# deepsphere/deepsphere-cosmo-tf2

Measured on AMD Instinct MI355X. Metric: Mpix*channels/s Chebyshev-conv fwd, nside=1024 K=5 F=64; HBM roofline %, higher is better.
Workload: dtype f32 (recurrence f32; contraction 3-pass split-bf16 MFMA with f32 accumulate; precision 'bf16x3' = the layer default for 64 input channels)

## Files before the change

deepsphere-cosmo-tf2_amd/csrc/cheb_fused.hip:

```cpp
#include <stdio.h>
#include <stdlib.h>
#include <string.h>

#include <algorithm>

#include "cheb_istrip_kernel.h"
#include "cheb_tiles.h"

namespace dsph {

void fused_images_begin(const dsph_plan* plan, const void* ws, uint64_t key, bool keep) {
  FusedPlan* fp = plan->fused;
  if (!fp || !ws) return;
  std::lock_guard<std::mutex> lock(fp->img_mu);
  if (fp->images.size() > 16384 && fp->images.find(ws) == fp->images.end()) fp->images.clear();
  FusedPlan::Images& im = fp->images[ws];
  if (!keep || im.key != key) { im.key = key; im.mask = 0; }
}
bool fused_images_claim(const dsph_plan* plan, const void* ws, uint32_t bit) {
  FusedPlan* fp = plan->fused;
  if (!fp || !ws) return true;
  std::lock_guard<std::mutex> lock(fp->img_mu);
  auto it = fp->images.find(ws);
  if (it == fp->images.end()) return true;
// ... 388 lines not shown

static int launch_strips(const FusedRequest& rq, const Route& rt, const WeightImages& img, const LaunchBase& base) {
  const dsph_plan* plan = rq.plan;
  const FusedTiles& ft = rt.ft;
  if (rt.strips == Strips::quad) {
    QStripLaunch qs;
    static_cast<LaunchBase&>(qs) = base;
    qs.wimg = rq.ws + img.qstrip;
    qs.strips = ft.q5.d_strips;
    qs.tab = ft.q5.d_tab;
    qs.prefix = ft.q5.d_prefix;
    qs.tape_rows = ft.q5.tape_rows;
    qs.nstrips = ft.q5.n; qs.Fin = rq.Fin; qs.Fout = rq.Fout;
    qs.f16 = rq.precision == DSPH_PREC_F16X3;
    qs.f16_xexp = plan->opt.f16_xexp;
    qs.prep_weights = fused_images_claim(plan, rq.ws, IMG_QSTRIP);
    return launch_cheb_qstrip(qs, rq.stream);
  }
  if (rt.strips == Strips::pairs) {
    StripLaunch st;
    static_cast<LaunchBase&>(st) = base;
    st.wimg = rq.ws + img.strip;
    st.pairs = ft.d_pairs;
    st.npairs = ft.n_pairs; st.Fin = rq.Fin; st.Fout = rq.Fout; st.K = rq.K; st.precision = struct_arithmetic(rq.precision);
    st.prep_weights = fused_images_claim(plan, rq.ws, IMG_STRIP);
    return launch_cheb_strip(st, rq.stream);
  }
  IStripLaunch is;
  static_cast<LaunchBase&>(is) = base;
  is.wimg = rq.ws + img.istrip;
// ... 389 lines not shown
```

deepsphere-cosmo-tf2_amd/csrc/cheb_qstrip.hip:

```cpp
#include <math.h>
#include <stdio.h>
#include <stdlib.h>

#include <algorithm>
#include <vector>

#include "cheb_qstrip_kernel.h"
#include "dsphere_wfrag.h"

namespace dsph {

__global__ __launch_bounds__(256) void qstrip_wprep_kernel(const float* __restrict__ w, unsigned char* __restrict__ out, int Fin,
                                                           int Fout, int cheb, int ld, int f16) {
  constexpr int K = 5;
  const int blk = blockIdx.x;
  const int kb = blk & 1, lev = (blk >> 1) % 3, oq = ((blk >> 1) / 3) & 3, role = (blk >> 1) / 12;
  const int j = role == 0 ? K - 1 - lev : 1 - lev;
  const bool have = role == 0 || lev < 2;
  float sc = qs_wsign(cheb != 0, j) * ((cheb != 0 && j == 0) ? 2.f : 1.f);
  if (f16) {
    const float pw = qt_wimg_pow2(w, Fin * K, Fout, ld);
    sc *= pw;
    if (blk == 0 && threadIdx.x == 0) *reinterpret_cast<float*>(out + (size_t)2 * 4 * 3 * 2 * 2 * QS_FRAG) = 1.f / pw;
  }
// ... 29 lines not shown
  return qtape_split(num_cu, tape_rows, N, mean_height, QS_RUNIN, grid, pieces, wg_per_piece);
}

size_t qstrip_wimg_bytes() { return (size_t)2 * 4 * 3 * 2 * 2 * QS_FRAG + 256; }

int launch_cheb_qstrip(const QStripLaunch& s, hipStream_t stream) {
  if (s.prep_weights) {
    hipLaunchKernelGGL(qstrip_wprep_kernel, dim3(2 * 4 * 3 * 2), dim3(256), 0, stream, s.w, s.wimg, (int)s.Fin, (int)s.Fout, s.cheb ? 1 : 0,
                       (int)s.ld, s.f16 ? 1 : 0);
    DSPH_HIP(hipGetLastError());
  }
  QStripArgs a;
  a.Fin = s.Fin;
  a.Fout = s.Fout;
  const int grid = qtape_forward_args(a, s, QS_RUNIN);
  void (*kern)(QStripArgs) = s.f16 ? (s.cheb ? cheb_qstrip5_kernel<true, true> : cheb_qstrip5_kernel<false, true>)
                                   : (s.cheb ? cheb_qstrip5_kernel<true, false> : cheb_qstrip5_kernel<false, false>);
#ifdef DSPH_QS_STAMPS
  static unsigned* d_stamps = nullptr;
  constexpr size_t NST = 8 * 4 * 10;
  if (!d_stamps) DSPH_HIP(hipMalloc(&d_stamps, NST * 4));
  DSPH_HIP(hipMemsetAsync(d_stamps, 0, NST * 4, stream));
  a.stamps = d_stamps;
#endif
  hipLaunchKernelGGL(kern, dim3(grid), dim3(QS_THREADS), 0, stream, a);
  DSPH_HIP(hipGetLastError());
#ifdef DSPH_QS_STAMPS
  if (getenv("DSPH_STAMPS_DUMP")) {
    std::vector<unsigned> h(NST);
    if (hipStreamSynchronize(stream) == hipSuccess && hipMemcpy(h.data(), d_stamps, NST * 4, hipMemcpyDeviceToHost) == hipSuccess)
      for (int w = 0; w < 8; ++w)
        for (int it = 0; it < 4; ++it) {
// ... 17 lines not shown
```

deepsphere-cosmo-tf2_amd/csrc/cheb_qstrip_kernel.h:

```cpp
#pragma once

#include <type_traits>

#include "cheb_qtape.h"

namespace dsph {

constexpr int QS_PX = 64;
constexpr int QS_D = 4;
constexpr int QS_USE = QS_PX - 2 * QS_D;
constexpr int QS_THREADS = 512;
constexpr int QS_RUNIN = 2 * QS_D + 1;

struct QStripArgs {
  const float* x;
  const float* bias;
  float* y;
  const unsigned char* wimg;
  const float* gvals8;
  const float* gdiag;
  const QStrip* strips;
  const int32_t* tab;
  const int32_t* prefix;
  int64_t x_rows, y_rows;
// ... 111 lines not shown
    qs_u12<INIT, NEG>(a0, a1, a2, a3, src.t[0][E], src.t[1][E], src.t[2][E], src.t[3][E], cw, cc, ce);                    \
    acc.t[0][E] = a0; acc.t[1][E] = a1; acc.t[2][E] = a2; acc.t[3][E] = a3;                                               \
  }
  if (e == 0) QS_UE(0)
  else if (e == 1) QS_UE(1)
  else if (e == 2) QS_UE(2)
  else QS_UE(3)
#undef QS_UE
}

#define QS_UPR 4
#define QS_UNIT qs_unit

__host__ __device__ constexpr float qs_wsign(bool cheb, int j) { return cheb && ((j & 3) >= 2) ? -1.f : 1.f; }

template <bool CHEB, bool F16>
__global__ __launch_bounds__(QS_THREADS, 2) void cheb_qstrip5_kernel(QStripArgs a) {
  constexpr int K = 5, D = QS_D, RING = K + 2;
#ifdef DSPH_QS_NOH1
  constexpr bool H1 = false;
#else
  constexpr bool H1 = CHEB;
#endif
  constexpr int ROWB = 2 * 2 * 4 * QS_FRAG;
  constexpr int RINGB = RING * ROWB;
  constexpr int HAND1 = 2 * 4 * QS_FRAG;
  constexpr int HANDB = 4 * HAND1;
  constexpr int CRING = K + 1;
  constexpr int CRINGB = CRING * QS_CROWB;
  constexpr int LDS_HAND = RINGB, LDS_C = RINGB + HANDB, LDS_FLAG = LDS_C + CRINGB;
  __shared__ __attribute__((aligned(16))) unsigned char smem[LDS_FLAG + 64];
// ... 30 lines not shown
  const unsigned x_goff = X_BY_H ? (unsigned)(2 * (lane >> 5) + (lane & 1)) * 16u
                                 : (unsigned)(lane >> 5) * 64u + (unsigned)(2 * ((lane >> 4) & 1) + (lane & 1)) * 16u;
  const unsigned x_loff = (unsigned)xt * QS_FRAG + (unsigned)(lane & 1) * 8u +
                          (X_BY_H ? (unsigned)(xpix + 16 * (lane >> 5)) * 16u : (unsigned)(xpix + 16 * (2 * (lane >> 5) + ((lane >> 4) & 1))) * 16u);
  auto tab_lane = [&](const QStrip& st, unsigned ci, int yrow) __attribute__((always_inline)) -> unsigned {
    return qt_tab_lane(a.tab, st, ci, min(max(yrow, st.ylo), st.yhi));
  };
  auto my_of = [&](int yrow) __attribute__((always_inline)) -> unsigned { return st_spread((unsigned)yrow & 15u) << 1; };
  auto my_next = [&](unsigned m) __attribute__((always_inline)) -> unsigned { return ((m | 0x55u) + 1u) & 0xaau; };
  auto xfetch = [&](const char* xmap, unsigned xrow, qs_f4 (&xv)[XN]) __attribute__((always_inline)) {
    if (QS_ABL & 8) {
#pragma unroll
      for (int i = 0; i < XN; ++i) xv[i] = qs_f4{0.f, 0.f, 0.f, 0.f};
      return;
    }
    const char* src = xmap + (size_t)(xrow * xrowb + x_goff);
#pragma unroll
    for (int i = 0; i < XN; ++i) xv[i] = *reinterpret_cast<const qs_f4*>(src + (X_BY_H ? 64 : 128) * i);
  };
  auto xw_wait = [&](qs_f4 (&xv)[XN]) __attribute__((always_inline)) {
    if (X_BY_H) asm volatile("" : "+v"(xv[0]), "+v"(xv[1]), "+v"(xv[XN - 2]), "+v"(xv[XN - 1]) : : "memory");
    else asm volatile("" : "+v"(xv[0]), "+v"(xv[1]) : : "memory");
  };
  auto xstore = [&](int slot, const qs_f4 (&xv)[XN]) __attribute__((always_inline)) {
    if (QS_ABL & 4096) {
#pragma unroll
      for (int i = 0; i < XN; ++i) asm volatile("" : : "v"(xv[i]));
      return;
    }
    unsigned char* q = smem + (unsigned)slot * ROWB + x_loff;
#pragma unroll
    for (int i = 0; i < XN; ++i) {
      const unsigned fo = X_BY_H ? (unsigned)(i >> 1) * (2 * 4 * QS_FRAG) + (unsigned)(i & 1) * (32u * 16u) : (unsigned)i * (2 * 4 * QS_FRAG);
      qs_u2 hi, lo;
#pragma unroll
      for (int j = 0; j < 2; ++j) {
        const float a0 = F16 ? xv[i][2 * j] * a.xsc : xv[i][2 * j], a1 = F16 ? xv[i][2 * j + 1] * a.xsc : xv[i][2 * j + 1];
        const qs_u2 hl = qt_split<F16>(a0, a1);
        hi[j] = hl[0];
        lo[j] = hl[1];
      }
      *reinterpret_cast<qs_u2*>(q + fo) = hi;
      *reinterpret_cast<qs_u2*>(q + fo + 4 * QS_FRAG) = lo;
    }
  };
  auto cfetch = [&](unsigned rid, qs_f4& cv, float& cd) __attribute__((always_inline)) { qt_cfetch(a.gvals8, a.gdiag, rid, q4, cv, cd); };
  auto cw_wait = [&](qs_f4& cv, float& cd) __attribute__((always_inline)) {
    asm volatile("" : "+v"(cv), "+v"(cd) : : "memory");
  };
  auto cstore = [&](int slot, qs_f4 cv, float cd) __attribute__((always_inline)) {
    if (CHEB) { cv = cv + cv; cd = cd + cd; }
    unsigned char* q = smem + LDS_C + (unsigned)slot * QS_CROWB + (unsigned)p * 16u + (unsigned)oq * 4u;
    if (q4 < 2) {
#pragma unroll
      for (int d = 0; d < 4; ++d) *reinterpret_cast<float*>(q + (unsigned)(1 + 4 * q4 + d) * 256u) = cv[d];
    }
    if (q4 == 2) *reinterpret_cast<float*>(q) = cd;
  };
  constexpr bool C_OFF = (QS_ABL & 1024) != 0;
  auto clo_read = [&](int slot) __attribute__((always_inline)) -> QCoefLo { return qt_clo_read<C_OFF>(smem + LDS_C, slot, p); };
  auto chi_read = [&](int slot) __attribute__((always_inline)) -> QCoefHi { return qt_chi_read<C_OFF>(smem + LDS_C, slot, p); };

#if QS_ABL & 512
#define QS_FRLOAD(P) (wr[0][0][0])
#else
#define QS_FRLOAD(P) (*reinterpret_cast<const qs_bf8*>(P))
#endif
#define QS_ORD_A(j) ((j) == 1 ? 1 : 0)
#define QS_ORD_B(j) ((j) == 0 ? 1 : 0)
#define QS_FR0(FADDR)                                                                                                     \
  _Pragma("unroll") for (int u = 0; u < 2; ++u) {                                                                         \
    fr[0][u][0] = QS_FRLOAD(smem + (FADDR) + (unsigned)u * QS_FRAG);                                                      \
    fr[0][u][1] = QS_FRLOAD(smem + (FADDR) + (unsigned)(4 + u) * QS_FRAG);                                                \
  }
#define QS_SETS(S0, S1, ROW, ZERO, WLEV, FADDR, NU, ...)                                                                  \
  _Pragma("unroll") for (int s = (S0); s < (S1); ++s) {                 \
    if (s + 1 < 4) {                                                                                                      \
      _Pragma("unroll") for (int u = 0; u < 2; ++u) {                                                                     \
        const unsigned fo = (unsigned)(((s + 1) >> 1) * 8 + ((s + 1) & 1) * 2 + u) * QS_FRAG;                             \
        fr[(s + 1) & 1][u][0] = QS_FRLOAD(smem + (FADDR) + fo);                                                           \
        fr[(s + 1) & 1][u][1] = QS_FRLOAD(smem + (FADDR) + fo + 4 * QS_FRAG);                                             \
      }                                                                                                                   \
    }                                                                                                                     \
    _Pragma("unroll") for (int j = 0; j < 3; ++j) {                                                                       \
      _Pragma("unroll") for (int u = 0; u < 2; ++u) {                                                                     \
        const int m = (s * 3 + j) * 2 + u;                                                                                \
        const int tt = (s & 1) * 2 + u;                                                                                   \
        const qs_bf8& wa_ = wr[WLEV][s >> 1][QS_ORD_A(j)];                                                                \
        const qs_bf8& bb_ = fr[s & 1][u][QS_ORD_B(j)];                                                                    \
        if ((ZERO) && s < 2 && j == 0) qs_m0<F16>((ROW).t[tt], wa_, bb_);                                                 \
        else qs_m<F16>((ROW).t[tt], wa_, bb_);                                                                            \
        _Pragma("unroll") for (int qq = (m * (NU)) / 18; qq < ((m + 1) * (NU)) / 18 && m < 18; ++qq) { __VA_ARGS__; }     \
      }                                                                                                                   \
    }                                                                                                                     \
  }
#define QS_CHAIN(ROW, ZERO, WLEV, FADDR, NU, TAIL, ...)                                                                   \
  {                                                                                                                       \
    QS_SETS(0, 3, ROW, ZERO, WLEV, FADDR, NU, __VA_ARGS__)                                                                \
// ... 10 lines not shown
#pragma unroll
      for (int kb = 0; kb < 2; ++kb)
#pragma unroll
        for (int h = 0; h < 2; ++h) wr[3][kb][h] = *reinterpret_cast<const qs_bf8*>(wp1 + (size_t)(kb * 2 + h) * QS_FRAG);
    }
    {
      const unsigned char* wp = a.wimg + ((size_t)(0 * 4 + oq) * 3) * (2 * 2 * QS_FRAG) + lane16;
#pragma unroll
      for (int l = 0; l < 3; ++l)
#pragma unroll
        for (int kb = 0; kb < 2; ++kb)
#pragma unroll
          for (int h = 0; h < 2; ++h) wr[l][kb][h] = *reinterpret_cast<const qs_bf8*>(wp + ((size_t)(l * 2 + kb) * 2 + h) * QS_FRAG);
    }
    int handed = 0;
    for (int64_t tr = tape.begin; tr < tape.end;) {
      QStrip st;
      tr += locate(tr, tape.end, st);
      for (int nq = wg.map0; nq < a.N; nq += a.wg_per_piece) {
      const int Xc = min(max(st.xs + 4 * p + oq, st.xlo), st.xhi);
      const int Xf = min(max(st.xs + 4 * xpix + xt, st.xlo), st.xhi);
      const int tc0 = max(st.xs, st.xlo) >> 4;
      const unsigned ciC = (unsigned)((Xc >> 4) - tc0), mXc = st_spread((unsigned)Xc & 15u);
      const unsigned ciF = (unsigned)((Xf >> 4) - tc0), mXf = st_spread((unsigned)Xf & 15u);
      const int T3 = ((st.y1 - st.y0) + 2 * D + 1 + 3) / 3;
      const char* __restrict__ xmap = reinterpret_cast<const char*>(a.x) + (size_t)nq * a.x_rows * xrowb;
      QRow R[2][3];
#pragma unroll
      for (int i = 0; i < 2; ++i)
#pragma unroll
        for (int s = 0; s < 3; ++s)
#pragma unroll
          for (int t = 0; t < 4; ++t) R[i][s].t[t] = qs_f4{0.f, 0.f, 0.f, 0.f};
      int ytop = st.y0 - D, slot_top = 0, cs_top = 0;
      qt_step_barrier();
      {
        qs_f4 cv, xv[XN];
        float cd;
        cfetch(qt_row_in(st, tab_lane(st, ciC, ytop - 1), mXc, ytop - 1), cv, cd);
        xfetch(xmap, qt_row_in(st, tab_lane(st, ciF, ytop), mXf, ytop), xv);
        cw_wait(cv, cd);
        cstore(CRING - 1, cv, cd);
        xw_wait(xv);
        xstore(0, xv);
      }
      unsigned bXf = tab_lane(st, ciF, ytop + 1), bXc = tab_lane(st, ciC, ytop);
      unsigned myX = my_of(ytop + 1), myC = my_of(ytop);
      qt_step_barrier();
      auto step = [&](auto ph_c) __attribute__((always_inline)) {
        constexpr int PH = decltype(ph_c)::value;
        constexpr int L0 = PH % 3, L1 = (PH + 1) % 3, L2 = (PH + 2) % 3;
        int snew = slot_top + 1;
        snew = snew == RING ? 0 : snew;
        auto slot_ix = [&](int back) __attribute__((always_inline)) -> int {
          int s = slot_top - back;
          s += s < 0 ? RING : 0;
          return s;
        };
        auto cslot_ix = [&](int back) __attribute__((always_inline)) -> int {
          int s = cs_top - back;
          s += s < 0 ? CRING : 0;
          return s;
        };
        QS_STAMP_DECL
        QS_STAMP(0);
        qs_f4 xv[XN];
        constexpr bool XLATE = H1;
        if (myX == 0) bXf = tab_lane(st, ciF, ytop + 1);
        if (myC == 0) bXc = tab_lane(st, ciC, ytop);
        if (!XLATE) xfetch(xmap, bXf + (mXf | myX), xv);
        const unsigned f0 = (unsigned)slot_top * ROWB + lane16, f1 = (unsigned)slot_ix(1) * ROWB + lane16, f2 = (unsigned)slot_ix(2) * ROWB + lane16;
        const unsigned f3 = (unsigned)slot_ix(3) * ROWB + lane16;
        constexpr bool N3 = CHEB;
        qs_bf8 fr[2][2][2];
        QCoefLo c3 = clo_read(cslot_ix(1));
        QS_FR0(f0)
        QCoefLo c2;
        QCoefHi c3h, c2h;
        qs_f4 cv;
        float cd;
        QS_CHAIN(R[0][L2], true, 0, f0, 2 * QS_UPR, { c2 = clo_read(cslot_ix(2)); QS_FR0(f1) },
                 { if (qq < QS_UPR) QS_UNIT<true, N3>(R[1][L2], R[0][L0], qq, QS_LO0(c3)); else QS_UNIT<false, N3>(R[1][L2], R[0][L1], qq - QS_UPR, QS_LO1(c3)); })
        qs_settle<9>(R[0][L2]);
        qs_settle<1>(R[1][L2]);
        QS_STAMP(1);
        QS_CHAIN(R[1][L2], false, 1, f1, 2 * QS_UPR, { c3h = chi_read(cslot_ix(1)); QS_FR0(f2) },
                 { if (qq < QS_UPR) QS_UNIT<!CHEB, false>(R[0][L0], R[1][L0], qq, QS_LO0(c2)); else QS_UNIT<false, false>(R[0][L0], R[1][L1], qq - QS_UPR, QS_LO1(c2)); })
        qs_settle<9>(R[1][L2]);
        qs_settle<1>(R[0][L0]);
        if (XLATE) xfetch(xmap, bXf + (mXf | myX), xv);
        QS_STAMP(2);
        QS_CHAIN(R[0][L0], false, 2, f2, QS_UPR, { c2h = chi_read(cslot_ix(2)); cfetch(bXc + (mXc | myC), cv, cd); if (H1) { QS_FR0(f3) } },
                 { QS_UNIT<false, N3>(R[1][L2], R[0][L2], qq, QS_HI(c3h)); })
        qs_settle<9>(R[0][L0]);
        qs_settle<1>(R[1][L2]);
        QS_STAMP(3);
        if (H1) {
          QS_CHAIN(R[1][L0], false, 3, f3, QS_UPR, {}, { QS_UNIT<false, false>(R[0][L0], R[1][L2], qq, QS_HI(c2h)); })
          qs_settle<9>(R[1][L0]);
        } else {
#pragma unroll
          for (int qq = 0; qq < QS_UPR; ++qq) QS_UNIT<false, false>(R[0][L0], R[1][L2], qq, QS_HI(c2h));
        }
        QS_STAMP(4);
        for (int spin = 0; flag_get() <= handed && spin < (1 << 22); ++spin) {}
        if (!(QS_ABL & 2048)) {
          unsigned char* hp = smem + hand;
#pragma unroll
          for (int t = 0; t < 4; ++t) {
            *reinterpret_cast<qs_f4*>(hp + t * QS_FRAG) = R[0][L0].t[t];
            if (CHEB) *reinterpret_cast<qs_f4*>(hp + (4 + t) * QS_FRAG) = R[1][L0].t[t];
          }
        }
        ++handed;
        QS_STAMP(5);
        xw_wait(xv);
        cw_wait(cv, cd);
        QS_STAMP(6);
        cstore(cs_top, cv, cd);
        xstore(snew, xv);
        QS_STAMP(7);
        slot_top = snew;
        cs_top = cs_top + 1 == CRING ? 0 : cs_top + 1;
        ++ytop;
        myX = my_next(myX);
        myC = my_next(myC);
        qt_step_barrier();
        QS_STAMP(8);
      };
      for (int t3 = 0; t3 < T3; ++t3) {
        step(std::integral_constant<int, 0>{});
        step(std::integral_constant<int, 1>{});
        step(std::integral_constant<int, 2>{});
      }
      }
    }
  } else {
    qs_bf8 wr[2][2][2];
    {
      const unsigned char* wp = a.wimg + ((size_t)(1 * 4 + oq) * 3) * (2 * 2 * QS_FRAG) + lane16;
#pragma unroll
// ... 23 lines not shown
      const int Xg = st.xs + 4 * p;
      const unsigned ciY = (unsigned)((min(max(Xg, st.xlo), st.xhi) >> 4) - tc0), mXg = st_spread((unsigned)Xg & 12u);
      const int cfirst = st.x0 - st.xs, clast = cfirst + st.w;
      const int T3 = ((st.y1 - st.y0) + 2 * D + 1 + 3) / 3;
      const char* __restrict__ xmap = reinterpret_cast<const char*>(a.x) + (size_t)nq * a.x_rows * xrowb;
      char* __restrict__ ymap = reinterpret_cast<char*>(a.y) + (size_t)nq * a.y_rows * yrowb;
      QRow R[2][3], Y;
#pragma unroll
      for (int i = 0; i < 2; ++i)
#pragma unroll
        for (int s = 0; s < 3; ++s)
#pragma unroll
          for (int t = 0; t < 4; ++t) R[i][s].t[t] = qs_f4{0.f, 0.f, 0.f, 0.f};
#pragma unroll
      for (int t = 0; t < 4; ++t) Y.t[t] = qs_f4{0.f, 0.f, 0.f, 0.f};
      int ytop = st.y0 - D, slot_top = 0, cs_top = 0;
      qt_step_barrier();
      if (!X_BY_H) {
        qs_f4 xv[XN];
        xfetch(xmap, qt_row_in(st, tab_lane(st, ciF, ytop), mXf, ytop), xv);
        xw_wait(xv);
        xstore(0, xv);
      }
      unsigned bXf = X_BY_H ? 0u : tab_lane(st, ciF, ytop + 1), bY = tab_lane(st, ciY, st.y0);
      unsigned myX = my_of(ytop + 1), myY = my_of(ytop - K);
      qt_step_barrier();
      auto step = [&](auto ph_c) __attribute__((always_inline)) {
        constexpr int PH = decltype(ph_c)::value;
        constexpr int L0 = PH % 3, L1 = (PH + 1) % 3, L2 = (PH + 2) % 3;
        int snew = slot_top + 1;
        snew = snew == RING ? 0 : snew;
        auto slot_ix = [&](int back) __attribute__((always_inline)) -> int {
          int s = slot_top - back;
          s += s < 0 ? RING : 0;
          return s;
        };
        auto cslot_ix = [&](int back) __attribute__((always_inline)) -> int {
          int s = cs_top - back;
          s += s < 0 ? CRING : 0;
          return s;
        };
        QS_STAMP_DECL
        QS_STAMP(0);
        qs_f4 xv[XN];
        if (!X_BY_H && myX == 0) bXf = tab_lane(st, ciF, ytop + 1);
        if (myY == 0) bY = tab_lane(st, ciY, ytop - K);
        if (!X_BY_H) xfetch(xmap, bXf + (mXf | myX), xv);
#ifdef DSPH_QS_LEARLY
        constexpr bool LE = CHEB && H1;
#else
        constexpr bool LE = false;
#endif
        QCoefLo c0;
        QCoefHi c0h;
        if (LE) c0 = clo_read(cslot_ix(5));
        if (!(QS_ABL & 2048)) {
          const unsigned char* hp = smem + hand;
#pragma unroll
          for (int t = 0; t < 4; ++t) {
            R[0][L2].t[t] = *reinterpret_cast<const qs_f4*>(hp + t * QS_FRAG);
            if (CHEB) R[1][L2].t[t] = *reinterpret_cast<const qs_f4*>(hp + (4 + t) * QS_FRAG);
          }
        }
        ++taken;
        flag_set(taken);
        const unsigned f1 = (unsigned)slot_ix(4) * ROWB + lane16, f0 = (unsigned)slot_ix(5) * ROWB + lane16;
        constexpr bool N1 = CHEB;
        QS_STAMP(1);
        qs_bf8 fr[2][2][2];
        if (LE) {
#pragma unroll
          for (int t = 0; t < 4; ++t) Y.t[t] = R[0][L0].t[t] + R[0][L0].t[t];
          qs_settle<1>(Y);
#pragma unroll
          for (int qq = 0; qq < 2 * QS_UPR; ++qq) {
            if (qq < QS_UPR) QS_UNIT<false, false>(Y, R[1][L0], qq, QS_LO0(c0)); else QS_UNIT<false, false>(Y, R[1][L1], qq - QS_UPR, QS_LO1(c0));
          }
          qs_settle<1>(Y);
        }
        const QCoefLo c1 = clo_read(cslot_ix(4));
        const QCoefHi c1h = chi_read(cslot_ix(4));
        QS_FR0(f0)
#ifdef DSPH_QS_LBARE
        if (CHEB && H1) {
          c0 = clo_read(cslot_ix(5));
          c0h = chi_read(cslot_ix(5));
#pragma unroll
          for (int qq = 0; qq < 3 * QS_UPR; ++qq) {
            if (qq < QS_UPR) QS_UNIT<false, N1>(R[1][L2], R[0][L0], qq, QS_LO0(c1));
            else if (qq < 2 * QS_UPR) QS_UNIT<false, N1>(R[1][L2], R[0][L1], qq - QS_UPR, QS_LO1(c1));
            else QS_UNIT<false, N1>(R[1][L2], R[0][L2], qq - 2 * QS_UPR, QS_HI(c1h));
          }
#pragma unroll
          for (int t = 0; t < 4; ++t) Y.t[t] = R[0][L0].t[t] + R[0][L0].t[t];
          qs_settle<1>(Y);
#pragma unroll
          for (int qq = 0; qq < 2 * QS_UPR; ++qq) {
            if (qq < QS_UPR) QS_UNIT<false, false>(Y, R[1][L0], qq, QS_LO0(c0)); else QS_UNIT<false, false>(Y, R[1][L1], qq - QS_UPR, QS_LO1(c0));
          }
          qs_settle<1>(R[1][L2]);
#pragma unroll
          for (int qq = 0; qq < QS_UPR; ++qq) QS_UNIT<false, false>(Y, R[1][L2], qq, QS_HI(c0h));
          qs_settle<1>(Y);
          QS_STAMP(2);
          QS_CHAIN(Y, false, 1, f0, 0, {}, {})
          qs_settle<9>(Y);
          QS_STAMP(3);
        } else
#endif
        {
        if (CHEB && !LE) {
#pragma unroll
          for (int t = 0; t < 4; ++t) Y.t[t] = R[0][L0].t[t] + R[0][L0].t[t];
          qs_settle<1>(Y);
        }
        QS_CHAIN(Y, !CHEB, 1, f0, 3 * QS_UPR, { if (!LE) c0 = clo_read(cslot_ix(5)); else c0h = chi_read(cslot_ix(5)); if (!H1) { QS_FR0(f1) } },
                 { if (qq < QS_UPR) QS_UNIT<!CHEB, N1>(R[1][L2], R[0][L0], qq, QS_LO0(c1));
                   else if (qq < 2 * QS_UPR) QS_UNIT<false, N1>(R[1][L2], R[0][L1], qq - QS_UPR, QS_LO1(c1));
                   else QS_UNIT<false, N1>(R[1][L2], R[0][L2], qq - 2 * QS_UPR, QS_HI(c1h)); })
        qs_settle<9>(Y);
        qs_settle<1>(R[1][L2]);
        QS_STAMP(2);
        if (H1 && LE) {
        } else if (H1) {
          c0h = chi_read(cslot_ix(5));
#pragma unroll
          for (int qq = 0; qq < 2 * QS_UPR; ++qq) {
            if (qq < QS_UPR) QS_UNIT<false, false>(Y, R[1][L0], qq, QS_LO0(c0)); else QS_UNIT<false, false>(Y, R[1][L1], qq - QS_UPR, QS_LO1(c0));
          }
        } else {
          QS_CHAIN(R[1][L2], false, 0, f1, 2 * QS_UPR, { c0h = chi_read(cslot_ix(5)); },
                   { if (qq < QS_UPR) QS_UNIT<false, false>(Y, R[1][L0], qq, QS_LO0(c0)); else QS_UNIT<false, false>(Y, R[1][L1], qq - QS_UPR, QS_LO1(c0)); })
        }
        qs_settle<9>(R[1][L2]);
        QS_STAMP(3);
#pragma unroll
        for (int qq = 0; qq < QS_UPR; ++qq) QS_UNIT<false, false>(Y, R[1][L2], qq, QS_HI(c0h));
        }
        QS_STAMP(4);
        if (!X_BY_H) xw_wait(xv);
        QS_STAMP(5);
        {
          const int yr = ytop - K;
          const bool row_ok = yr >= st.y0 && yr < ((QS_ABL & 16) ? st.y0 + 1 : st.y1);
          const unsigned rowg = bY + (mXg | myY);
#pragma unroll
          for (int t = 0; t < 4; ++t) {
            const int c = 4 * p + t;
            if (row_ok && c >= cfirst && c < clast) {
              qs_f4 o;
#pragma unroll
              for (int e = 0; e < 4; ++e) {
                const float v = fmaf(Y.t[t][e], ysc, bv[e]);
                o[e] = F16 ? (v < floor_v ? floor_v : v) : fmaxf(v, floor_v);
              }
              *reinterpret_cast<qs_f4*>(ymap + (size_t)(rowg + (unsigned)((t & 1) + 4 * (t >> 1))) * yrowb + (unsigned)(16 * oq + 4 * q4) * 4u) = o;
            }
          }
        }
        QS_STAMP(6);
        if (!X_BY_H) xstore(snew, xv);
        QS_STAMP(7);
        slot_top = snew;
        cs_top = cs_top + 1 == CRING ? 0 : cs_top + 1;
        ++ytop;
        myX = my_next(myX);
        myY = my_next(myY);
        qt_step_barrier();
        QS_STAMP(8);
      };
      for (int t3 = 0; t3 < T3; ++t3) {
        step(std::integral_constant<int, 0>{});
        step(std::integral_constant<int, 1>{});
        step(std::integral_constant<int, 2>{});
      }
      }
    }
  }
#undef QS_CHAIN
// ... 7 lines not shown
```

deepsphere-cosmo-tf2_amd/csrc/dsphere_api.hip:

```cpp
#include <stdarg.h>
#include <stdio.h>
#include <string.h>

#include <new>

#include "dsphere_common.h"

namespace dsph {

static thread_local char g_err[512] = "";

void set_error(const char* fmt, ...) {
  va_list ap;
  va_start(ap, fmt);
  vsnprintf(g_err, sizeof(g_err), fmt, ap);
  va_end(ap);
}

int hip_fail(hipError_t e, const char* what) {
  set_error("HIP error %d (%s) in %s", (int)e, hipGetErrorString(e), what);
  return DSPH_E_HIP;
}

static size_t align_up(size_t v, size_t a) { return (v + a - 1) / a * a; }
// ... 120 lines not shown
      if (value < 0 || value > 2) { set_error("plan_set_option: DSPH_OPT_SPLIT takes 0 (automatic), 1 (always), 2 (never)"); return DSPH_E_BADARG; }
      o.split_order = (int)value;
      tables = false;
      break;
    case DSPH_OPT_TSTEP: o.tstep = value != 0; tables = false; break;
    case DSPH_OPT_PACK: o.pack = value != 0; tables = false; break;
    case DSPH_OPT_STRIP_FORM:
      if (value < 0 || value > 1) { set_error("plan_set_option: DSPH_OPT_STRIP_FORM takes 0 (quad strips) or 1 (strip pairs)"); return DSPH_E_BADARG; }
      o.strip_form = (int)value;
      break;
    case DSPH_OPT_F16_XEXP:
      if (value < -100 || value > 100) { set_error("plan_set_option: DSPH_OPT_F16_XEXP takes a binary exponent in [-100, 100]"); return DSPH_E_BADARG; }
      o.f16_xexp = (int)value;
      tables = false;
      break;
    default: set_error("plan_set_option: unknown option %d", (int)option); return DSPH_E_BADARG;
  }
  if (tables && p->fused) {
    if (fused_host_released(p->fused)) {
      set_error("plan_set_option: the plan's host copy of L~ was released (DSPH_PREPARE_RELEASE_HOST); set options before preparing");
      return DSPH_E_UNSUPPORTED;
    }
    DeviceGuard guard(p->device);
    fused_plan_invalidate(p->fused);
  }
  p->opt = o;
  return DSPH_OK;
}

int dsph_plan_strip_pairs(const dsph_plan* p, int32_t K, int32_t* out, int64_t capacity, int64_t* n_pairs) {
// ... 404 lines not shown
```

deepsphere-cosmo-tf2_amd/csrc/dsphere_common.h:

```cpp
#pragma once

#include <hip/hip_runtime.h>
#include <stdint.h>

#include <vector>

#include "dsphere.h"

namespace dsph {

void set_error(const char* fmt, ...);
int hip_fail(hipError_t e, const char* what);

#define DSPH_HIP(call)                                           \
  do {                                                           \
    hipError_t e__ = (call);                                     \
    if (e__ != hipSuccess) return ::dsph::hip_fail(e__, #call);  \
  } while (0)

struct DeviceGuard {
  int prev = -1;
  bool ok = true;
  explicit DeviceGuard(int dev) {
    if (hipGetDevice(&prev) != hipSuccess) { ok = false; return; }
// ... 5 lines not shown
};

struct FusedPlan;

struct PlanOptions {
  int strips = 0;
  bool use_struct = true;
  bool use_tables = true;
  bool fork = true;
  int strip_min_rows = 4;
  int split_order = 0;
  bool tstep = true;
  int strip_form = 0;
  bool pack = true;
  int f16_xexp = 0;
};

}

struct dsph_plan {
  int device = 0;
  int64_t n_rows = 0;
  int64_t n_cols = 0;
  int32_t width = 0;
  int32_t* d_cols = nullptr;
  float* d_vals = nullptr;
  std::vector<int64_t> levels;
  dsph::PlanOptions opt;
  dsph::FusedPlan* fused = nullptr;
};
// ... 134 lines not shown
struct QTapeLaunch : LaunchBase {
  unsigned char* wimg;
  const QStrip* strips;
  const int32_t* tab = nullptr;
  const int32_t* prefix;
  int64_t tape_rows;
  int32_t nstrips;
  bool f16 = false;
  int f16_xexp = 0;
  bool prep_weights = true;
};
int64_t qtape_split(int num_cu, int64_t tape_rows, int64_t N, int64_t mean_height, int run_in, int* grid, int* pieces, int* wg_per_piece);

struct QStripLaunch : QTapeLaunch {
  int32_t Fin, Fout;
};
bool qstrip_shape_ok(int32_t Fin, int32_t Fout, int32_t K);
size_t qstrip_wimg_bytes();
int64_t qstrip_split(int num_cu, int64_t tape_rows, int64_t N, int64_t mean_height, int* grid, int* pieces, int* wg_per_piece);
int launch_cheb_qstrip(const QStripLaunch& s, hipStream_t stream);

struct QStrip8Launch : QTapeLaunch {
  int32_t ld_w;
};
bool qstrip8_shape_ok(int32_t Fin, int32_t Fout, int32_t K);
size_t qstrip8_wimg_bytes();
int64_t qstrip8_split(int num_cu, int64_t tape_rows, int64_t N, int64_t mean_height, int* grid, int* pieces, int* wg_per_piece);
int launch_cheb_qstrip8(const QStrip8Launch& s, hipStream_t stream);

struct QWgradLaunch {
// ... 57 lines not shown
```

deepsphere-cosmo-tf2_amd/deepsphere/_native.py:

```python

import ctypes
import os

import numpy as np

_LIB_PATH = os.path.join(os.path.dirname(os.path.abspath(__file__)), "_lib", "libdsphere_hip.so")
_lib = None

OK = 0
ACT_NONE, ACT_RELU, ACT_ELU, ACT_SIGMOID, ACT_TANH = 0, 1, 2, 3, 4
PREC_FP32, PREC_BF16X3, PREC_BF16X6, PREC_F16X3 = 0, 1, 2, 3
ALGO_AUTO, ALGO_UNFUSED, ALGO_FUSED = 0, 1, 2
PART_ALL, PART_INTERIOR, PART_BOUNDARY = 0, 1, 2
FWD_KEEP_WEIGHTS = 1
ABI_VERSION = 3
POOL_MAX, POOL_AVG = 0, 1
PREPARE_BACKWARD, PREPARE_RELEASE_HOST = 1, 2
BASIS_CHEBYSHEV, BASIS_MONOMIAL = 0, 1
OPT_STRIPS, OPT_STRUCT, OPT_TABLES, OPT_FORK, OPT_STRIP_MINROWS, OPT_SPLIT, OPT_TSTEP = 1, 2, 3, 4, 6, 8, 9
OPT_PACK = 10
OPT_STRIP_FORM = 11
OPT_F16_XEXP = 12
STRIP_FORM_QUAD, STRIP_FORM_PAIRS = 0, 1
STRIPS_AUTO, STRIPS_ALWAYS, STRIPS_NEVER = 0, 1, 2
SPLIT_AUTO, SPLIT_ALWAYS, SPLIT_NEVER = 0, 1, 2

_c_i64 = ctypes.c_int64
_c_i32 = ctypes.c_int32
_c_vp = ctypes.c_void_p

SIGNATURES = {
    "dsph_abi_version": (ctypes.c_int, []),
    "dsph_last_error": (ctypes.c_char_p, []),
    "dsph_plan_create": (ctypes.c_int, [ctypes.POINTER(_c_vp), _c_i64, _c_i64, _c_i32, _c_vp, _c_vp, ctypes.c_int]),
    "dsph_plan_destroy": (None, [_c_vp]),
    "dsph_plan_set_levels": (ctypes.c_int, [_c_vp, _c_i32, _c_vp]),
    "dsph_plan_set_option": (ctypes.c_int, [_c_vp, _c_i32, _c_i64]),
# ... 990 lines not shown
```

include/dsphere.h:

```cpp
#ifndef DSPHERE_H
#define DSPHERE_H

#include <stddef.h>
#include <stdint.h>

#ifdef __cplusplus
extern "C" {
#endif

#define DSPH_ABI_VERSION 3

#define DSPH_OK 0
#define DSPH_E_BADARG (-1)
#define DSPH_E_HIP (-2)
#define DSPH_E_UNSUPPORTED (-3)
#define DSPH_E_WORKSPACE (-4)

#define DSPH_ACT_NONE 0
#define DSPH_ACT_RELU 1
#define DSPH_ACT_ELU 2
#define DSPH_ACT_SIGMOID 3
#define DSPH_ACT_TANH 4

#define DSPH_PREC_FP32 0
// ... 20 lines not shown
#define DSPH_PREPARE_BACKWARD 1
#define DSPH_PREPARE_RELEASE_HOST 2
int dsph_plan_prepare(dsph_plan* plan, int32_t K, int32_t Fin, int32_t flags);
int dsph_plan_prepare_layer(dsph_plan* plan, int32_t K, int32_t Fin, int32_t Fout, int32_t flags);

#define DSPH_OPT_STRIPS 1
#define DSPH_OPT_STRUCT 2
#define DSPH_OPT_TABLES 3
#define DSPH_OPT_FORK 4
#define DSPH_OPT_STRIP_MINROWS 6
#define DSPH_OPT_SPLIT 8
#define DSPH_OPT_TSTEP 9
#define DSPH_OPT_PACK 10
#define DSPH_OPT_STRIP_FORM 11
#define DSPH_OPT_F16_XEXP 12
int dsph_plan_set_option(dsph_plan* plan, int32_t option, int64_t value);

int64_t dsph_plan_rows(const dsph_plan* plan);
int64_t dsph_plan_cols(const dsph_plan* plan);
int32_t dsph_plan_ell_width(const dsph_plan* plan);
int64_t dsph_plan_out_rows(const dsph_plan* plan, int32_t K);
int dsph_plan_fused_ok(const dsph_plan* plan, int32_t Fin, int32_t Fout, int32_t K);
int dsph_plan_uses_chain(const dsph_plan* plan, int32_t Fin, int32_t Fout, int32_t K);

int dsph_plan_tile_counts(const dsph_plan* plan, int32_t K, int64_t* n_struct, int64_t* n_bfs);

int dsph_plan_strip_tiles(const dsph_plan* plan, int64_t N, int32_t Fin, int32_t Fout, int32_t K, int32_t precision,
                          int64_t* n_tiles);

int dsph_plan_strip_pairs(const dsph_plan* plan, int32_t K, int32_t* out, int64_t capacity, int64_t* n_pairs);
// ... 144 lines not shown
```

Measured before the change: 301,900.

## Use 32-bit addressing and rotating ring offsets in quad-strip Chebyshev kernel

Adds a template flag so the quad-strip kernel computes global x, coefficient and y addresses with 32-bit unsigned offsets when tensors fit in 4 GiB, with a 64-bit fallback selected on the host or forced by a new plan option. Ring-slot indices are replaced by precomputed byte offsets rotated each step, removing the per-step modulo arithmetic. It also adds readfirstlane on the spin flag, moves the lane-derived values for the recurrence base into hand-managed registers, and rewrites the output store with hoisted column masks. The goal is to cut scalar and vector address ALU work and register pressure in the inner step. The cost is more kernel variants and layout assumptions such as a 256-byte row stride in the 32-bit path.

Result: no change. 304,600 (median of 6 runs) (+0.9%).

```diff
diff --git a/deepsphere-cosmo-tf2_amd/csrc/cheb_fused.hip b/deepsphere-cosmo-tf2_amd/csrc/cheb_fused.hip
--- a/deepsphere-cosmo-tf2_amd/csrc/cheb_fused.hip
+++ b/deepsphere-cosmo-tf2_amd/csrc/cheb_fused.hip
@@ -426,6 +426,7 @@
     qs.nstrips = ft.q5.n; qs.Fin = rq.Fin; qs.Fout = rq.Fout;
     qs.f16 = rq.precision == DSPH_PREC_F16X3;
     qs.f16_xexp = plan->opt.f16_xexp;
+    qs.addr64 = plan->opt.qstrip_addr64;
     qs.prep_weights = fused_images_claim(plan, rq.ws, IMG_QSTRIP);
     return launch_cheb_qstrip(qs, rq.stream);
   }
diff --git a/deepsphere-cosmo-tf2_amd/csrc/cheb_qstrip.hip b/deepsphere-cosmo-tf2_amd/csrc/cheb_qstrip.hip
--- a/deepsphere-cosmo-tf2_amd/csrc/cheb_qstrip.hip
+++ b/deepsphere-cosmo-tf2_amd/csrc/cheb_qstrip.hip
@@ -67,8 +67,14 @@
   a.Fin = s.Fin;
   a.Fout = s.Fout;
   const int grid = qtape_forward_args(a, s, QS_RUNIN);
-  void (*kern)(QStripArgs) = s.f16 ? (s.cheb ? cheb_qstrip5_kernel<true, true> : cheb_qstrip5_kernel<false, true>)
-                                   : (s.cheb ? cheb_qstrip5_kernel<true, false> : cheb_qstrip5_kernel<false, false>);
+  const uint64_t lim = (uint64_t)1 << 32;
+  const bool a64 = s.addr64 || (uint64_t)s.x_rows * (uint64_t)s.Fin * 4u >= lim || (uint64_t)s.y_rows * (uint64_t)s.ld * 4u >= lim ||
+                   (uint64_t)s.x_rows * 32u >= lim;
+  void (*kern)(QStripArgs) =
+      a64 ? (s.f16 ? (s.cheb ? cheb_qstrip5_kernel<true, true, true> : cheb_qstrip5_kernel<false, true, true>)
+                   : (s.cheb ? cheb_qstrip5_kernel<true, false, true> : cheb_qstrip5_kernel<false, false, true>))
+          : (s.f16 ? (s.cheb ? cheb_qstrip5_kernel<true, true, false> : cheb_qstrip5_kernel<false, true, false>)
+                   : (s.cheb ? cheb_qstrip5_kernel<true, false, false> : cheb_qstrip5_kernel<false, false, false>));
 #ifdef DSPH_QS_STAMPS
   static unsigned* d_stamps = nullptr;
   constexpr size_t NST = 8 * 4 * 10;
diff --git a/deepsphere-cosmo-tf2_amd/csrc/cheb_qstrip_kernel.h b/deepsphere-cosmo-tf2_amd/csrc/cheb_qstrip_kernel.h
--- a/deepsphere-cosmo-tf2_amd/csrc/cheb_qstrip_kernel.h
+++ b/deepsphere-cosmo-tf2_amd/csrc/cheb_qstrip_kernel.h
@@ -149,7 +149,7 @@
 
 __host__ __device__ constexpr float qs_wsign(bool cheb, int j) { return cheb && ((j & 3) >= 2) ? -1.f : 1.f; }
 
-template <bool CHEB, bool F16>
+template <bool CHEB, bool F16, bool A64>
 __global__ __launch_bounds__(QS_THREADS, 2) void cheb_qstrip5_kernel(QStripArgs a) {
   constexpr int K = 5, D = QS_D, RING = K + 2;
 #ifdef DSPH_QS_NOH1
@@ -210,7 +210,7 @@
       for (int i = 0; i < XN; ++i) xv[i] = qs_f4{0.f, 0.f, 0.f, 0.f};
       return;
     }
-    const char* src = xmap + (size_t)(xrow * xrowb + x_goff);
+    const char* src = A64 ? xmap + ((size_t)xrow * xrowb + x_goff) : xmap + (size_t)((xrow << 8) | x_goff);
 #pragma unroll
     for (int i = 0; i < XN; ++i) xv[i] = *reinterpret_cast<const qs_f4*>(src + (X_BY_H ? 64 : 128) * i);
   };
@@ -218,13 +218,13 @@
     if (X_BY_H) asm volatile("" : "+v"(xv[0]), "+v"(xv[1]), "+v"(xv[XN - 2]), "+v"(xv[XN - 1]) : : "memory");
     else asm volatile("" : "+v"(xv[0]), "+v"(xv[1]) : : "memory");
   };
-  auto xstore = [&](int slot, const qs_f4 (&xv)[XN]) __attribute__((always_inline)) {
+  auto xstore = [&](unsigned xo, const qs_f4 (&xv)[XN]) __attribute__((always_inline)) {
     if (QS_ABL & 4096) {
 #pragma unroll
       for (int i = 0; i < XN; ++i) asm volatile("" : : "v"(xv[i]));
       return;
     }
-    unsigned char* q = smem + (unsigned)slot * ROWB + x_loff;
+    unsigned char* q = smem + xo + x_loff;
 #pragma unroll
     for (int i = 0; i < XN; ++i) {
       const unsigned fo = X_BY_H ? (unsigned)(i >> 1) * (2 * 4 * QS_FRAG) + (unsigned)(i & 1) * (32u * 16u) : (unsigned)i * (2 * 4 * QS_FRAG);
@@ -240,22 +240,26 @@
       *reinterpret_cast<qs_u2*>(q + fo + 4 * QS_FRAG) = lo;
     }
   };
-  auto cfetch = [&](unsigned rid, qs_f4& cv, float& cd) __attribute__((always_inline)) { qt_cfetch(a.gvals8, a.gdiag, rid, q4, cv, cd); };
+  auto cfetch = [&](unsigned rid, qs_f4& cv, float& cd) __attribute__((always_inline)) {
+    if (A64) { qt_cfetch(a.gvals8, a.gdiag, rid, q4, cv, cd); return; }
+    cv = *reinterpret_cast<const qs_f4*>(reinterpret_cast<const char*>(a.gvals8) + (size_t)((rid << 5) | ((unsigned)(q4 & 1) << 4)));
+    cd = *reinterpret_cast<const float*>(reinterpret_cast<const char*>(a.gdiag) + (size_t)(rid << 2));
+  };
   auto cw_wait = [&](qs_f4& cv, float& cd) __attribute__((always_inline)) {
     asm volatile("" : "+v"(cv), "+v"(cd) : : "memory");
   };
-  auto cstore = [&](int slot, qs_f4 cv, float cd) __attribute__((always_inline)) {
+  auto cstore = [&](unsigned co, unsigned c_cvoff, qs_f4 cv, float cd) __attribute__((always_inline)) {
     if (CHEB) { cv = cv + cv; cd = cd + cd; }
-    unsigned char* q = smem + LDS_C + (unsigned)slot * QS_CROWB + (unsigned)p * 16u + (unsigned)oq * 4u;
-    if (q4 < 2) {
-#pragma unroll
-      for (int d = 0; d < 4; ++d) *reinterpret_cast<float*>(q + (unsigned)(1 + 4 * q4 + d) * 256u) = cv[d];
-    }
-    if (q4 == 2) *reinterpret_cast<float*>(q) = cd;
+    unsigned char* q = smem + LDS_C + (co + (unsigned)oq * 4u) + (unsigned)p * 16u;
+#pragma unroll
+    for (int d = 0; d < 4; ++d) *reinterpret_cast<float*>(q + c_cvoff + (unsigned)d * 256u) = cv[d];
+    *reinterpret_cast<float*>(q) = cd;
   };
   constexpr bool C_OFF = (QS_ABL & 1024) != 0;
-  auto clo_read = [&](int slot) __attribute__((always_inline)) -> QCoefLo { return qt_clo_read<C_OFF>(smem + LDS_C, slot, p); };
-  auto chi_read = [&](int slot) __attribute__((always_inline)) -> QCoefHi { return qt_chi_read<C_OFF>(smem + LDS_C, slot, p); };
+  auto clo_read = [&](unsigned co) __attribute__((always_inline)) -> QCoefLo { return qt_clo_read<C_OFF>(smem + LDS_C + co, 0, p); };
+  auto chi_read = [&](unsigned co) __attribute__((always_inline)) -> QCoefHi { return qt_chi_read<C_OFF>(smem + LDS_C + co, 0, p); };
+  auto x_wrap = [&](unsigned xo) __attribute__((always_inline)) -> unsigned { return xo + ROWB == (unsigned)RINGB ? 0u : xo + ROWB; };
+  auto c_wrap = [&](unsigned co) __attribute__((always_inline)) -> unsigned { return co + QS_CROWB == (unsigned)CRINGB ? 0u : co + QS_CROWB; };
 
 #if QS_ABL & 512
 #define QS_FRLOAD(P) (wr[0][0][0])
@@ -278,6 +282,8 @@
         fr[(s + 1) & 1][u][1] = QS_FRLOAD(smem + (FADDR) + fo + 4 * QS_FRAG);                                             \
       }                                                                                                                   \
     }                                                                                                                     \
+          \
+    asm volatile("" : : "v"(fr[s & 1][0][0]), "v"(fr[s & 1][0][1]), "v"(fr[s & 1][1][0]), "v"(fr[s & 1][1][1]));            \
     _Pragma("unroll") for (int j = 0; j < 3; ++j) {                                                                       \
       _Pragma("unroll") for (int u = 0; u < 2; ++u) {                                                                     \
         const int m = (s * 3 + j) * 2 + u;                                                                                \
@@ -318,12 +324,16 @@
           for (int h = 0; h < 2; ++h) wr[l][kb][h] = *reinterpret_cast<const qs_bf8*>(wp + ((size_t)(l * 2 + kb) * 2 + h) * QS_FRAG);
     }
     int handed = 0;
+    const unsigned c_cvoff = (unsigned)(1 + 4 * (q4 & 1)) * 256u;
     for (int64_t tr = tape.begin; tr < tape.end;) {
       QStrip st;
       tr += locate(tr, tape.end, st);
       for (int nq = wg.map0; nq < a.N; nq += a.wg_per_piece) {
-      const int Xc = min(max(st.xs + 4 * p + oq, st.xlo), st.xhi);
-      const int Xf = min(max(st.xs + 4 * xpix + xt, st.xlo), st.xhi);
+      int ln = lane;
+      asm volatile("" : "+v"(ln));
+      const int p_s = ln & 15, xpix_s = X_BY_H ? ((ln >> 1) & 15) : (((ln >> 1) & 7) + 8 * (wave >> 2));
+      const int Xc = min(max(st.xs + 4 * p_s + oq, st.xlo), st.xhi);
+      const int Xf = min(max(st.xs + 4 * xpix_s + xt, st.xlo), st.xhi);
       const int tc0 = max(st.xs, st.xlo) >> 4;
       const unsigned ciC = (unsigned)((Xc >> 4) - tc0), mXc = st_spread((unsigned)Xc & 15u);
       const unsigned ciF = (unsigned)((Xf >> 4) - tc0), mXf = st_spread((unsigned)Xf & 15u);
@@ -336,7 +346,10 @@
         for (int s = 0; s < 3; ++s)
 #pragma unroll
           for (int t = 0; t < 4; ++t) R[i][s].t[t] = qs_f4{0.f, 0.f, 0.f, 0.f};
-      int ytop = st.y0 - D, slot_top = 0, cs_top = 0;
+      int ytop = st.y0 - D;
+      unsigned xo0 = 0, xo1 = 6 * ROWB, xo2 = 5 * ROWB, xo3 = 4 * ROWB;
+      unsigned co1 = 5 * QS_CROWB, co2 = 4 * QS_CROWB;
+      asm volatile("" : "+s"(co1));
       qt_step_barrier();
       {
         qs_f4 cv, xv[XN];
@@ -344,57 +357,48 @@
         cfetch(qt_row_in(st, tab_lane(st, ciC, ytop - 1), mXc, ytop - 1), cv, cd);
         xfetch(xmap, qt_row_in(st, tab_lane(st, ciF, ytop), mXf, ytop), xv);
         cw_wait(cv, cd);
-        cstore(CRING - 1, cv, cd);
+        cstore(co1, c_cvoff, cv, cd);
         xw_wait(xv);
-        xstore(0, xv);
+        xstore(xo0, xv);
       }
-      unsigned bXf = tab_lane(st, ciF, ytop + 1), bXc = tab_lane(st, ciC, ytop);
+      auto base_of = [&](int X, int yrow) __attribute__((always_inline)) -> unsigned {
+        asm volatile("" : "+v"(X));
+        return tab_lane(st, (unsigned)((X >> 4) - tc0), yrow) + st_spread((unsigned)X & 15u);
+      };
+      unsigned bXf = base_of(Xf, ytop + 1), bXc = base_of(Xc, ytop);
       unsigned myX = my_of(ytop + 1), myC = my_of(ytop);
       qt_step_barrier();
       auto step = [&](auto ph_c) __attribute__((always_inline)) {
         constexpr int PH = decltype(ph_c)::value;
         constexpr int L0 = PH % 3, L1 = (PH + 1) % 3, L2 = (PH + 2) % 3;
-        int snew = slot_top + 1;
-        snew = snew == RING ? 0 : snew;
-        auto slot_ix = [&](int back) __attribute__((always_inline)) -> int {
-          int s = slot_top - back;
-          s += s < 0 ? RING : 0;
-          return s;
-        };
-        auto cslot_ix = [&](int back) __attribute__((always_inline)) -> int {
-          int s = cs_top - back;
-          s += s < 0 ? CRING : 0;
-          return s;
-        };
         QS_STAMP_DECL
         QS_STAMP(0);
         qs_f4 xv[XN];
         constexpr bool XLATE = H1;
-        if (myX == 0) bXf = tab_lane(st, ciF, ytop + 1);
-        if (myC == 0) bXc = tab_lane(st, ciC, ytop);
-        if (!XLATE) xfetch(xmap, bXf + (mXf | myX), xv);
-        const unsigned f0 = (unsigned)slot_top * ROWB + lane16, f1 = (unsigned)slot_ix(1) * ROWB + lane16, f2 = (unsigned)slot_ix(2) * ROWB + lane16;
-        const unsigned f3 = (unsigned)slot_ix(3) * ROWB + lane16;
+        if (myX == 0) bXf = base_of(Xf, ytop + 1);
+        if (myC == 0) bXc = base_of(Xc, ytop);
+        if (!XLATE) xfetch(xmap, bXf + myX, xv);
+        const unsigned f0 = xo0 + lane16, f1 = xo1 + lane16, f2 = xo2 + lane16, f3 = xo3 + lane16;
         constexpr bool N3 = CHEB;
         qs_bf8 fr[2][2][2];
-        QCoefLo c3 = clo_read(cslot_ix(1));
+        QCoefLo c3 = clo_read(co1);
         QS_FR0(f0)
         QCoefLo c2;
         QCoefHi c3h, c2h;
         qs_f4 cv;
         float cd;
-        QS_CHAIN(R[0][L2], true, 0, f0, 2 * QS_UPR, { c2 = clo_read(cslot_ix(2)); QS_FR0(f1) },
+        QS_CHAIN(R[0][L2], true, 0, f0, 2 * QS_UPR, { c2 = clo_read(co2); QS_FR0(f1) },
                  { if (qq < QS_UPR) QS_UNIT<true, N3>(R[1][L2], R[0][L0], qq, QS_LO0(c3)); else QS_UNIT<false, N3>(R[1][L2], R[0][L1], qq - QS_UPR, QS_LO1(c3)); })
         qs_settle<9>(R[0][L2]);
         qs_settle<1>(R[1][L2]);
         QS_STAMP(1);
-        QS_CHAIN(R[1][L2], false, 1, f1, 2 * QS_UPR, { c3h = chi_read(cslot_ix(1)); QS_FR0(f2) },
+        QS_CHAIN(R[1][L2], false, 1, f1, 2 * QS_UPR, { c3h = chi_read(co1); QS_FR0(f2) },
                  { if (qq < QS_UPR) QS_UNIT<!CHEB, false>(R[0][L0], R[1][L0], qq, QS_LO0(c2)); else QS_UNIT<false, false>(R[0][L0], R[1][L1], qq - QS_UPR, QS_LO1(c2)); })
         qs_settle<9>(R[1][L2]);
         qs_settle<1>(R[0][L0]);
-        if (XLATE) xfetch(xmap, bXf + (mXf | myX), xv);
+        if (XLATE) xfetch(xmap, bXf + myX, xv);
         QS_STAMP(2);
-        QS_CHAIN(R[0][L0], false, 2, f2, QS_UPR, { c2h = chi_read(cslot_ix(2)); cfetch(bXc + (mXc | myC), cv, cd); if (H1) { QS_FR0(f3) } },
+        QS_CHAIN(R[0][L0], false, 2, f2, QS_UPR, { c2h = chi_read(co2); cfetch(bXc + myC, cv, cd); if (H1) { QS_FR0(f3) } },
                  { QS_UNIT<false, N3>(R[1][L2], R[0][L2], qq, QS_HI(c3h)); })
         qs_settle<9>(R[0][L0]);
         qs_settle<1>(R[1][L2]);
@@ -407,7 +411,7 @@
           for (int qq = 0; qq < QS_UPR; ++qq) QS_UNIT<false, false>(R[0][L0], R[1][L2], qq, QS_HI(c2h));
         }
         QS_STAMP(4);
-        for (int spin = 0; flag_get() <= handed && spin < (1 << 22); ++spin) {}
+        for (int spin = 0; __builtin_amdgcn_readfirstlane(flag_get()) <= handed && spin < (1 << 22); ++spin) {}
         if (!(QS_ABL & 2048)) {
           unsigned char* hp = smem + hand;
 #pragma unroll
@@ -421,14 +425,15 @@
         xw_wait(xv);
         cw_wait(cv, cd);
         QS_STAMP(6);
-        cstore(cs_top, cv, cd);
-        xstore(snew, xv);
+        const unsigned co0 = c_wrap(co1), xon = x_wrap(xo0);
+        cstore(co0, c_cvoff, cv, cd);
+        xstore(xon, xv);
         QS_STAMP(7);
-        slot_top = snew;
-        cs_top = cs_top + 1 == CRING ? 0 : cs_top + 1;
+        xo3 = xo2; xo2 = xo1; xo1 = xo0; xo0 = xon;
+        co2 = co1; co1 = co0;
         ++ytop;
+        myC = myX;
         myX = my_next(myX);
-        myC = my_next(myC);
         qt_step_barrier();
         QS_STAMP(8);
       };
@@ -482,38 +487,33 @@
           for (int t = 0; t < 4; ++t) R[i][s].t[t] = qs_f4{0.f, 0.f, 0.f, 0.f};
 #pragma unroll
       for (int t = 0; t < 4; ++t) Y.t[t] = qs_f4{0.f, 0.f, 0.f, 0.f};
-      int ytop = st.y0 - D, slot_top = 0, cs_top = 0;
+      int ytop = st.y0 - D;
+      unsigned xo4 = 3 * ROWB, xo5 = 2 * ROWB, xon = ROWB;
+      unsigned co4 = 2 * QS_CROWB, co5 = 1 * QS_CROWB;
+      const bool col_all = 4 * p >= cfirst && 4 * p + 3 < clast;
+      bool col_part[4];
+#pragma unroll
+      for (int t = 0; t < 4; ++t) col_part[t] = !col_all && 4 * p + t >= cfirst && 4 * p + t < clast;
+      const bool any_part = __builtin_amdgcn_ballot_w64(col_part[0] || col_part[1] || col_part[2] || col_part[3]) != 0;
       qt_step_barrier();
       if (!X_BY_H) {
         qs_f4 xv[XN];
         xfetch(xmap, qt_row_in(st, tab_lane(st, ciF, ytop), mXf, ytop), xv);
         xw_wait(xv);
-        xstore(0, xv);
+        xstore(0u, xv);
       }
-      unsigned bXf = X_BY_H ? 0u : tab_lane(st, ciF, ytop + 1), bY = tab_lane(st, ciY, st.y0);
+      unsigned bXf = X_BY_H ? 0u : tab_lane(st, ciF, ytop + 1) + mXf, bY = tab_lane(st, ciY, st.y0) + mXg;
       unsigned myX = my_of(ytop + 1), myY = my_of(ytop - K);
       qt_step_barrier();
       auto step = [&](auto ph_c) __attribute__((always_inline)) {
         constexpr int PH = decltype(ph_c)::value;
         constexpr int L0 = PH % 3, L1 = (PH + 1) % 3, L2 = (PH + 2) % 3;
-        int snew = slot_top + 1;
-        snew = snew == RING ? 0 : snew;
-        auto slot_ix = [&](int back) __attribute__((always_inline)) -> int {
-          int s = slot_top - back;
-          s += s < 0 ? RING : 0;
-          return s;
-        };
-        auto cslot_ix = [&](int back) __attribute__((always_inline)) -> int {
-          int s = cs_top - back;
-          s += s < 0 ? CRING : 0;
-          return s;
-        };
         QS_STAMP_DECL
         QS_STAMP(0);
         qs_f4 xv[XN];
-        if (!X_BY_H && myX == 0) bXf = tab_lane(st, ciF, ytop + 1);
-        if (myY == 0) bY = tab_lane(st, ciY, ytop - K);
-        if (!X_BY_H) xfetch(xmap, bXf + (mXf | myX), xv);
+        if (!X_BY_H && myX == 0) bXf = tab_lane(st, ciF, ytop + 1) + mXf;
+        if (myY == 0) bY = tab_lane(st, ciY, ytop - K) + mXg;
+        if (!X_BY_H) xfetch(xmap, bXf + myX, xv);
 #ifdef DSPH_QS_LEARLY
         constexpr bool LE = CHEB && H1;
 #else
@@ -521,7 +521,7 @@
 #endif
         QCoefLo c0;
         QCoefHi c0h;
-        if (LE) c0 = clo_read(cslot_ix(5));
+        if (LE) c0 = clo_read(co5);
         if (!(QS_ABL & 2048)) {
           const unsigned char* hp = smem + hand;
 #pragma unroll
@@ -532,7 +532,7 @@
         }
         ++taken;
         flag_set(taken);
-        const unsigned f1 = (unsigned)slot_ix(4) * ROWB + lane16, f0 = (unsigned)slot_ix(5) * ROWB + lane16;
+        const unsigned f1 = xo4 + lane16, f0 = xo5 + lane16;
         constexpr bool N1 = CHEB;
         QS_STAMP(1);
         qs_bf8 fr[2][2][2];
@@ -546,13 +546,13 @@
           }
           qs_settle<1>(Y);
         }
-        const QCoefLo c1 = clo_read(cslot_ix(4));
-        const QCoefHi c1h = chi_read(cslot_ix(4));
+        const QCoefLo c1 = clo_read(co4);
+        const QCoefHi c1h = chi_read(co4);
         QS_FR0(f0)
 #ifdef DSPH_QS_LBARE
         if (CHEB && H1) {
-          c0 = clo_read(cslot_ix(5));
-          c0h = chi_read(cslot_ix(5));
+          c0 = clo_read(co5);
+          c0h = chi_read(co5);
 #pragma unroll
           for (int qq = 0; qq < 3 * QS_UPR; ++qq) {
             if (qq < QS_UPR) QS_UNIT<false, N1>(R[1][L2], R[0][L0], qq, QS_LO0(c1));
@@ -582,7 +582,7 @@
           for (int t = 0; t < 4; ++t) Y.t[t] = R[0][L0].t[t] + R[0][L0].t[t];
           qs_settle<1>(Y);
         }
-        QS_CHAIN(Y, !CHEB, 1, f0, 3 * QS_UPR, { if (!LE) c0 = clo_read(cslot_ix(5)); else c0h = chi_read(cslot_ix(5)); if (!H1) { QS_FR0(f1) } },
+        QS_CHAIN(Y, !CHEB, 1, f0, 3 * QS_UPR, { if (!LE) c0 = clo_read(co5); else c0h = chi_read(co5); if (!H1) { QS_FR0(f1) } },
                  { if (qq < QS_UPR) QS_UNIT<!CHEB, N1>(R[1][L2], R[0][L0], qq, QS_LO0(c1));
                    else if (qq < 2 * QS_UPR) QS_UNIT<false, N1>(R[1][L2], R[0][L1], qq - QS_UPR, QS_LO1(c1));
                    else QS_UNIT<false, N1>(R[1][L2], R[0][L2], qq - 2 * QS_UPR, QS_HI(c1h)); })
@@ -591,13 +591,13 @@
         QS_STAMP(2);
         if (H1 && LE) {
         } else if (H1) {
-          c0h = chi_read(cslot_ix(5));
+          c0h = chi_read(co5);
 #pragma unroll
           for (int qq = 0; qq < 2 * QS_UPR; ++qq) {
             if (qq < QS_UPR) QS_UNIT<false, false>(Y, R[1][L0], qq, QS_LO0(c0)); else QS_UNIT<false, false>(Y, R[1][L1], qq - QS_UPR, QS_LO1(c0));
           }
         } else {
-          QS_CHAIN(R[1][L2], false, 0, f1, 2 * QS_UPR, { c0h = chi_read(cslot_ix(5)); },
+          QS_CHAIN(R[1][L2], false, 0, f1, 2 * QS_UPR, { c0h = chi_read(co5); },
                    { if (qq < QS_UPR) QS_UNIT<false, false>(Y, R[1][L0], qq, QS_LO0(c0)); else QS_UNIT<false, false>(Y, R[1][L1], qq - QS_UPR, QS_LO1(c0)); })
         }
         qs_settle<9>(R[1][L2]);
@@ -611,26 +611,40 @@
         {
           const int yr = ytop - K;
           const bool row_ok = yr >= st.y0 && yr < ((QS_ABL & 16) ? st.y0 + 1 : st.y1);
-          const unsigned rowg = bY + (mXg | myY);
-#pragma unroll
-          for (int t = 0; t < 4; ++t) {
-            const int c = 4 * p + t;
-            if (row_ok && c >= cfirst && c < clast) {
-              qs_f4 o;
+          const unsigned rowg = bY + myY;
+          if (row_ok) {
+            qs_f4 o[4];
+#pragma unroll
+            for (int t = 0; t < 4; ++t)
 #pragma unroll
               for (int e = 0; e < 4; ++e) {
                 const float v = fmaf(Y.t[t][e], ysc, bv[e]);
-                o[e] = F16 ? (v < floor_v ? floor_v : v) : fmaxf(v, floor_v);
+                o[t][e] = F16 ? (v < floor_v ? floor_v : v) : fmaxf(v, floor_v);
               }
-              *reinterpret_cast<qs_f4*>(ymap + (size_t)(rowg + (unsigned)((t & 1) + 4 * (t >> 1))) * yrowb + (unsigned)(16 * oq + 4 * q4) * 4u) = o;
+            const unsigned ycol = (unsigned)(16 * oq + 4 * q4) * 4u;
+            unsigned yo = rowg * yrowb + ycol;
+            if (!A64) asm volatile("" : "+v"(yo));
+            auto ystore = [&](int t) __attribute__((always_inline)) {
+              const unsigned dr = (unsigned)((t & 1) + 4 * (t >> 1));
+              if (A64) *reinterpret_cast<qs_f4*>(ymap + (size_t)(rowg + dr) * yrowb + ycol) = o[t];
+              else *reinterpret_cast<qs_f4*>(ymap + (size_t)(yo + dr * yrowb)) = o[t];
+            };
+            if (__builtin_expect(col_all, 1)) {
+#pragma unroll
+              for (int t = 0; t < 4; ++t) ystore(t);
+            }
+            if (any_part) {
+#pragma unroll
+              for (int t = 0; t < 4; ++t)
+                if (col_part[t]) ystore(t);
             }
           }
         }
         QS_STAMP(6);
-        if (!X_BY_H) xstore(snew, xv);
+        if (!X_BY_H) xstore(xon, xv);
         QS_STAMP(7);
-        slot_top = snew;
-        cs_top = cs_top + 1 == CRING ? 0 : cs_top + 1;
+        xo5 = xo4; xo4 = x_wrap(xo4); xon = x_wrap(xon);
+        co5 = co4; co4 = c_wrap(co4);
         ++ytop;
         myX = my_next(myX);
         myY = my_next(myY);
diff --git a/deepsphere-cosmo-tf2_amd/csrc/dsphere_api.hip b/deepsphere-cosmo-tf2_amd/csrc/dsphere_api.hip
--- a/deepsphere-cosmo-tf2_amd/csrc/dsphere_api.hip
+++ b/deepsphere-cosmo-tf2_amd/csrc/dsphere_api.hip
@@ -158,6 +158,7 @@
       o.f16_xexp = (int)value;
       tables = false;
       break;
+    case DSPH_OPT_QSTRIP_ADDR64: o.qstrip_addr64 = value != 0; tables = false; break;
     default: set_error("plan_set_option: unknown option %d", (int)option); return DSPH_E_BADARG;
   }
   if (tables && p->fused) {
diff --git a/deepsphere-cosmo-tf2_amd/csrc/dsphere_common.h b/deepsphere-cosmo-tf2_amd/csrc/dsphere_common.h
--- a/deepsphere-cosmo-tf2_amd/csrc/dsphere_common.h
+++ b/deepsphere-cosmo-tf2_amd/csrc/dsphere_common.h
@@ -43,6 +43,7 @@
   int strip_form = 0;
   bool pack = true;
   int f16_xexp = 0;
+  bool qstrip_addr64 = false;
 };
 
 }
@@ -207,6 +208,7 @@
 
 struct QStripLaunch : QTapeLaunch {
   int32_t Fin, Fout;
+  bool addr64 = false;
 };
 bool qstrip_shape_ok(int32_t Fin, int32_t Fout, int32_t K);
 size_t qstrip_wimg_bytes();
diff --git a/deepsphere-cosmo-tf2_amd/deepsphere/_native.py b/deepsphere-cosmo-tf2_amd/deepsphere/_native.py
--- a/deepsphere-cosmo-tf2_amd/deepsphere/_native.py
+++ b/deepsphere-cosmo-tf2_amd/deepsphere/_native.py
@@ -21,6 +21,7 @@
 OPT_PACK = 10
 OPT_STRIP_FORM = 11
 OPT_F16_XEXP = 12
+OPT_QSTRIP_ADDR64 = 13
 STRIP_FORM_QUAD, STRIP_FORM_PAIRS = 0, 1
 STRIPS_AUTO, STRIPS_ALWAYS, STRIPS_NEVER = 0, 1, 2
 SPLIT_AUTO, SPLIT_ALWAYS, SPLIT_NEVER = 0, 1, 2
diff --git a/include/dsphere.h b/include/dsphere.h
--- a/include/dsphere.h
+++ b/include/dsphere.h
@@ -58,6 +58,7 @@
 #define DSPH_OPT_PACK 10
 #define DSPH_OPT_STRIP_FORM 11
 #define DSPH_OPT_F16_XEXP 12
+#define DSPH_OPT_QSTRIP_ADDR64 13
 int dsph_plan_set_option(dsph_plan* plan, int32_t option, int64_t value);
 
 int64_t dsph_plan_rows(const dsph_plan* plan);
```
